# nikolovjovan/exblas

Measured on AMD Instinct MI355X. Metric: ExSUM fp64 Gelem/s at n=2^28 (bit-exact vs CPU superaccumulator/MPFR), higher is better.
Workload: dtype f64; 1 GPU; ExSUM n=2^28 fp64 ill_cond(c=1e+32), fpe=8 early_exit=True, 1xMI355X, inputs resident in HBM, steps rotate over 4 distinct vectors; n_total=268435456, fpe=8, early_exit=True, parallelism=single

## Files before the change

### exblas_amd/csrc/blas1.hip

```cpp
#include "superacc.hip.h"
#include "fpe.hip.h"
#include "exblas_internal.h"
#include <hip/hip_ext.h>

namespace exb {

constexpr int BLOCK = 256;
constexpr int WAVES = BLOCK / 64;

template <int N, bool EE, int COPIES, int CNT, int ZM = 0>
__device__ __forceinline__ void fpe_absorb(double (&a)[N > 0 ? N : 1], double (&x)[CNT], int from,
                                           long long *col, unsigned &flags)
{
    LdsSink<COPIES> sink{col, flags};
    fpe_absorb_sink<N, EE, CNT, LdsSink<COPIES>, ZM>(a, x, from, sink);
}

template <int N, int COPIES>
__device__ __forceinline__ void fpe_flush(double (&a)[N > 0 ? N : 1], long long *col, unsigned &flags)
{
    LdsSink<COPIES> sink{col, flags};
    fpe_flush_sink<N>(a, sink);
}

template <int COPIES>
__device__ __forceinline__ void block_epilogue(long long *s_acc, unsigned flags, long long *gacc,
                                               unsigned *gflags, int ngroups)
{
    __shared__ unsigned s_flags;
    if (threadIdx.x == 0) s_flags = 0;
    __syncthreads();
    if (flags) atomicOr(&s_flags, flags);
    long long *g = gacc + (size_t)(blockIdx.x % ngroups) * NL;
    for (int l = threadIdx.x; l < NL; l += BLOCK) {
        long long sum = 0;
#pragma unroll
        for (int w = 0; w < WAVES; ++w)
#pragma unroll
            for (int c = 0; c < COPIES; ++c) sum += s_acc[(w * NL + l) * COPIES + c];
        if (sum != 0) atomicAdd((unsigned long long *)&g[l], (unsigned long long)sum);
    }
    __syncthreads();
    if (threadIdx.x == 0 && s_flags) atomicOr(gflags, s_flags);
}

template <int N, bool EE, int COPIES, int U, bool NT, bool PF, int ZM = 0>
__global__ void __launch_bounds__(BLOCK) k_exsum(const double *__restrict__ a, long long n,
                                                 long long *__restrict__ gacc,
                                                 unsigned *__restrict__ gflags, int ngroups, int chunked)
{
    __shared__ long long s_acc[WAVES * NL * COPIES];
    auto zero_lds = [&]() {
        for (int i = threadIdx.x; i < WAVES * NL * COPIES; i += BLOCK) s_acc[i] = 0;
        __syncthreads();
    };
    const int wave = threadIdx.x >> 6, lane = threadIdx.x & 63;
    long long *col = s_acc + wave * NL * COPIES + (lane & (COPIES - 1));
    unsigned flags = 0;
    double fpe[N > 0 ? N : 1];
#pragma unroll
    for (int i = 0; i < (N > 0 ? N : 1); ++i) fpe[i] = 0.0;

    const long long head = (((uintptr_t)a & 8u) && n > 0) ? 1 : 0;
    const d2_t *v = (const d2_t *)(a + head);
    const long long nv = (n - head) >> 1;
    constexpr long long TILE = (long long)BLOCK * U;
    const long long ntiles = nv / TILE;
    LdsSink<COPIES> sinkm{col, flags};
    Bypass bypass;

    if constexpr (!PF) {
        zero_lds();
        for (long long t = blockIdx.x; t < ntiles; t += gridDim.x) {
            const d2_t *p = v + t * TILE + threadIdx.x;
            d2_t r[U];
#pragma unroll
            for (int u = 0; u < U; ++u) r[u] = ld2<NT>(p + u * BLOCK);
            double x[2 * U];
#pragma unroll
            for (int u = 0; u < U; ++u) {
                x[2 * u] = r[u].x;
                x[2 * u + 1] = r[u].y;
            }
            fpe_absorb_adaptive<N, EE, 2 * U, LdsSink<COPIES>, ZM>(fpe, x, sinkm, bypass);
        }
    } else {
        long long t = blockIdx.x, tstride = gridDim.x, tend = ntiles;
        if (chunked) {
            const long long per = (ntiles + gridDim.x - 1) / gridDim.x;
            t = blockIdx.x * per;
            tstride = 1;
            tend = min(ntiles, t + per);
        }
        if (t < tend) {
            d2_t r0[U], r1[U];
            auto fill = [&](long long tile, d2_t (&r)[U]) {
                const d2_t *p = v + (tile < tend ? tile : tend - 1) * TILE + threadIdx.x;
#pragma unroll
                for (int u = 0; u < U; ++u) r[u] = ld2<NT>(p + u * BLOCK);
            };
            auto absorb = [&](d2_t (&r)[U]) {
                double x[2 * U];
#pragma unroll
                for (int u = 0; u < U; ++u) {
                    x[2 * u] = r[u].x;
                    x[2 * u + 1] = r[u].y;
                }
                fpe_absorb_adaptive<N, EE, 2 * U, LdsSink<COPIES>, ZM>(fpe, x, sinkm, bypass);
            };
            fill(t, r0);
            zero_lds();
            for (;;) {
                fill(t + tstride, r1);
                absorb(r0);
                t += tstride;
                if (t >= tend) break;
                fill(t + tstride, r0);
                absorb(r1);
                t += tstride;
                if (t >= tend) break;
            }
        } else {
            zero_lds();
        }
    }
    for (long long i = ntiles * TILE + (long long)blockIdx.x * BLOCK + threadIdx.x; i < nv;
         i += (long long)gridDim.x * BLOCK) {
        d2_t r = v[i];
        double x[2] = {r.x, r.y};
        fpe_absorb<N, false, COPIES, 2>(fpe, x, 0, col, flags);
    }
    if (blockIdx.x == 0 && threadIdx.x == 0) {
        if (head) lds_add<COPIES>(col, a[0], flags);
        if ((n - head) & 1) lds_add<COPIES>(col, a[n - 1], flags);
    }
    fpe_flush<N, COPIES>(fpe, col, flags);
    block_epilogue<COPIES>(s_acc, flags, gacc, gflags, ngroups);
}

template <int N, bool EE, int COPIES>
__global__ void __launch_bounds__(BLOCK) k_exsum_strided(const double *__restrict__ a, long long n,
                                                         long long inca, long long *__restrict__ gacc,
                                                         unsigned *__restrict__ gflags, int ngroups)
{
    __shared__ long long s_acc[WAVES * NL * COPIES];
    for (int i = threadIdx.x; i < WAVES * NL * COPIES; i += BLOCK) s_acc[i] = 0;
    __syncthreads();
    const int wave = threadIdx.x >> 6, lane = threadIdx.x & 63;
    long long *col = s_acc + wave * NL * COPIES + (lane & (COPIES - 1));
    unsigned flags = 0;
    double fpe[N > 0 ? N : 1];
#pragma unroll
    for (int i = 0; i < (N > 0 ? N : 1); ++i) fpe[i] = 0.0;
    const long long T = (long long)gridDim.x * BLOCK;
    for (long long i = (long long)blockIdx.x * BLOCK + threadIdx.x; i < n; i += 4 * T) {
        double x[4];
#pragma unroll
        for (int u = 0; u < 4; ++u) x[u] = i + u * T < n ? a[(i + u * T) * inca] : 0.0;
        fpe_absorb<N, false, COPIES, 4>(fpe, x, 0, col, flags);
    }
    fpe_flush<N, COPIES>(fpe, col, flags);
    block_epilogue<COPIES>(s_acc, flags, gacc, gflags, ngroups);
}

template <int N, bool EE, int COPIES, int U, bool NT, bool PF, int WPS = 1, bool HALVES = false, int ZM = 0>
__global__ void __launch_bounds__(BLOCK, WPS) k_exdot(const double *__restrict__ a, const double *__restrict__ b,
                                                 long long n, long long *__restrict__ gacc,
                                                 unsigned *__restrict__ gflags, int ngroups)
{
    __shared__ long long s_acc[WAVES * NL * COPIES];
    auto zero_lds = [&]() {
        for (int i = threadIdx.x; i < WAVES * NL * COPIES; i += BLOCK) s_acc[i] = 0;
        __syncthreads();
    };
    const int wave = threadIdx.x >> 6, lane = threadIdx.x & 63;
    long long *col = s_acc + wave * NL * COPIES + (lane & (COPIES - 1));
    unsigned flags = 0;
    LdsSink<COPIES> sink{col, flags};
    long long *const lo_acc = low_acc_of(gflags), *const hi_acc = high_acc_of(gflags);
    double fpe[N > 0 ? N : 1];
#pragma unroll
    for (int i = 0; i < (N > 0 ? N : 1); ++i) fpe[i] = 0.0;

    const d2_t *va = (const d2_t *)a, *vb = (const d2_t *)b;
    const long long nv = n >> 1;
    Bypass bypass;
    constexpr long long TILE = (long long)BLOCK * U;
    const long long ntiles = nv / TILE;
    if constexpr (!PF) {
        zero_lds();
        for (long long t = blockIdx.x; t < ntiles; t += gridDim.x) {
            const long long base = t * TILE + threadIdx.x;
            d2_t ra[U], rb[U];
#pragma unroll
            for (int u = 0; u < U; ++u) {
                ra[u] = ld2<NT>(va + base + u * BLOCK);
                rb[u] = ld2<NT>(vb + base + u * BLOCK);
            }
            double x[2 * U], e[2 * U];
#pragma unroll
            for (int u = 0; u < U; ++u) {
                x[2 * u] = two_prod(ra[u].x, rb[u].x, e[2 * u]);
                x[2 * u + 1] = two_prod(ra[u].y, rb[u].y, e[2 * u + 1]);
            }
            if (!prod_range_divert<2 * U>(fpe[0], x, e, sink, lo_acc, hi_acc, [&](int j) { return j & 1 ? ra[j >> 1].y : ra[j >> 1].x; },
                                              [&](int j) { return j & 1 ? rb[j >> 1].y : rb[j >> 1].x; }))
                fpe_absorb_prod_adaptive<N, EE, 2 * U, LdsSink<COPIES>, 0, false>(fpe, x, e, sink, bypass);
        }
    } else {
        long long t = blockIdx.x;
        d2_t ra[U], rb[U];
        if (t < ntiles) {
            const long long base = t * TILE + threadIdx.x;
#pragma unroll
            for (int u = 0; u < U; ++u) {
                ra[u] = ld2<NT>(va + base + u * BLOCK);
                rb[u] = ld2<NT>(vb + base + u * BLOCK);
            }
        }
        zero_lds();
        if constexpr (HALVES) {
            while (t < ntiles) {
                const long long tn = t + gridDim.x;
                constexpr int H = U / 2;
#pragma unroll
                for (int h = 0; h < 2; ++h) {
                    double x[2 * H], e[2 * H];
#pragma unroll
                    for (int u = 0; u < H; ++u) {
                        x[2 * u] = two_prod(ra[h * H + u].x, rb[h * H + u].x, e[2 * u]);
                        x[2 * u + 1] = two_prod(ra[h * H + u].y, rb[h * H + u].y, e[2 * u + 1]);
                    }
                    const bool diverted = prod_range_divert<2 * H>(fpe[0], x, e, sink, lo_acc, hi_acc, [&](int j) { return j & 1 ? ra[h * H + (j >> 1)].y : ra[h * H + (j >> 1)].x; },
                        [&](int j) { return j & 1 ? rb[h * H + (j >> 1)].y : rb[h * H + (j >> 1)].x; });
                    if (tn < ntiles) {
                        const long long base = tn * TILE + threadIdx.x;
#pragma unroll
                        for (int u = 0; u < H; ++u) {
                            ra[h * H + u] = ld2<NT>(va + base + (h * H + u) * BLOCK);
                            rb[h * H + u] = ld2<NT>(vb + base + (h * H + u) * BLOCK);
                        }
                    }
                    if (!diverted) fpe_absorb_prod_adaptive<N, EE, 2 * H, LdsSink<COPIES>, 0, false>(fpe, x, e, sink, bypass);
                }
                t = tn;
            }
        } else if (t < ntiles) {
            d2_t rc[U], rd[U];
            auto fill = [&](long long tile, d2_t (&pa)[U], d2_t (&pb)[U]) {
                const long long base = (tile < ntiles ? tile : ntiles - 1) * TILE + threadIdx.x;
#pragma unroll
                for (int u = 0; u < U; ++u) {
                    pa[u] = ld2<NT>(va + base + u * BLOCK);
                    pb[u] = ld2<NT>(vb + base + u * BLOCK);
                }
            };
            auto absorb = [&](d2_t (&pa)[U], d2_t (&pb)[U]) {
                double x[2 * U], e[2 * U];
#pragma unroll
                for (int u = 0; u < U; ++u) {
                    x[2 * u] = two_prod(pa[u].x, pb[u].x, e[2 * u]);
                    x[2 * u + 1] = two_prod(pa[u].y, pb[u].y, e[2 * u + 1]);
                }
                if (!prod_range_divert<2 * U>(fpe[0], x, e, sink, lo_acc, hi_acc, [&](int j) { return j & 1 ? pa[j >> 1].y : pa[j >> 1].x; },
                                                  [&](int j) { return j & 1 ? pb[j >> 1].y : pb[j >> 1].x; }))
                    fpe_absorb_prod_adaptive<N, EE, 2 * U, LdsSink<COPIES>, ZM, false>(fpe, x, e, sink, bypass);
            };
            for (;;) {
                fill(t + gridDim.x, rc, rd);
                absorb(ra, rb);
                t += gridDim.x;
                if (t >= ntiles) break;
                fill(t + gridDim.x, ra, rb);
                absorb(rc, rd);
                t += gridDim.x;
                if (t >= ntiles) break;
            }
        }
    }
    for (long long i = ntiles * TILE + (long long)blockIdx.x * BLOCK + threadIdx.x; i < nv;
         i += (long long)gridDim.x * BLOCK) {
        d2_t ra = va[i], rb = vb[i];
        double x[2], e[2];
        x[0] = two_prod(ra.x, rb.x, e[0]);
        x[1] = two_prod(ra.y, rb.y, e[1]);
        if (!prod_range_divert<2>(fpe[0], x, e, sink, lo_acc, hi_acc, [&](int j) { return j ? ra.y : ra.x; }, [&](int j) { return j ? rb.y : rb.x; }))
            fpe_absorb_prod<N, false, 2, LdsSink<COPIES>, 0, false>(fpe, x, e, sink);
    }
    if (blockIdx.x == 0 && threadIdx.x == 0 && (n & 1)) {
        double x1[1], e1[1];
        x1[0] = two_prod(a[n - 1], b[n - 1], e1[0]);
        if (!prod_range_divert<1>(fpe[0], x1, e1, sink, lo_acc, hi_acc, [&](int) { return a[n - 1]; }, [&](int) { return b[n - 1]; }))
            sink_product(sink, x1[0], e1[0]);
    }
    fpe_flush<N, COPIES>(fpe, col, flags);
    block_epilogue<COPIES>(s_acc, flags, gacc, gflags, ngroups);
}

template <int N, bool EE, int COPIES>
__global__ void __launch_bounds__(BLOCK) k_exdot_strided(const double *__restrict__ a, long long inca,
                                                         const double *__restrict__ b, long long incb,
                                                         long long n, long long *__restrict__ gacc,
                                                         unsigned *__restrict__ gflags, int ngroups)
{
    __shared__ long long s_acc[WAVES * NL * COPIES];
    for (int i = threadIdx.x; i < WAVES * NL * COPIES; i += BLOCK) s_acc[i] = 0;
    __syncthreads();
    const int wave = threadIdx.x >> 6, lane = threadIdx.x & 63;
    long long *col = s_acc + wave * NL * COPIES + (lane & (COPIES - 1));
    unsigned flags = 0;
    LdsSink<COPIES> sink{col, flags};
    long long *const lo_acc = low_acc_of(gflags), *const hi_acc = high_acc_of(gflags);
    double fpe[N > 0 ? N : 1];
#pragma unroll
    for (int i = 0; i < (N > 0 ? N : 1); ++i) fpe[i] = 0.0;
    const long long T = (long long)gridDim.x * BLOCK;
    for (long long i = (long long)blockIdx.x * BLOCK + threadIdx.x; i < n; i += 4 * T) {
        double va[4], vb[4], x[4], e[4];
#pragma unroll
        for (int u = 0; u < 4; ++u) {
            const bool in = i + u * T < n;
            va[u] = in ? a[(i + u * T) * inca] : 0.0;
            vb[u] = in ? b[(i + u * T) * incb] : 0.0;
        }
#pragma unroll
        for (int u = 0; u < 4; ++u) x[u] = two_prod(va[u], vb[u], e[u]);
        if (!prod_range_divert<4>(fpe[0], x, e, sink, lo_acc, hi_acc, [&](int j) { return va[j]; }, [&](int j) { return vb[j]; }))
            fpe_absorb_prod<N, false, 4, LdsSink<COPIES>, 0, false>(fpe, x, e, sink);
    }
    fpe_flush<N, COPIES>(fpe, col, flags);
    block_epilogue<COPIES>(s_acc, flags, gacc, gflags, ngroups);
}

__global__ void __launch_bounds__(64) k_finalize(long long *sets, int nsets, int set_stride, unsigned *gflags,
                                                 unsigned flags_or, int zero_sets, long long *out,
                                                 const long long *ext_in, long long *ext_out)
{
    const int lane = threadIdx.x;
    unsigned flags = flags_or;
    if (gflags) flags |= *gflags;
    if (set_stride >= SET_WORDS) {
        for (int g = 0; g < nsets; ++g)
        {
            for (int k = 0; k < 3; ++k)
                if (sets[(size_t)g * set_stride + NL + k] != 0) flags |= (1u << k);
            const long long pw = sets[(size_t)g * set_stride + NL + 3];
            if (pw & 0xffff) flags |= FLAG_PUNDER;
            if (pw >> 16) flags |= FLAG_POVER;
        }
    }
    long long lo0 = 0, hi0 = 0, lo1 = 0, hi1 = 0;
    for (int g0 = 0; g0 < nsets; g0 += 16) {
        long long t0[16], t1[16];
#pragma unroll
        for (int k = 0; k < 16; ++k) {
            const bool ok = g0 + k < nsets;
            const long long *p = sets + (size_t)(ok ? g0 + k : 0) * set_stride;
            t0[k] = ok ? __builtin_nontemporal_load(p + lane) : 0;
            t1[k] = (ok && lane < NL - 64) ? __builtin_nontemporal_load(p + 64 + lane) : 0;
        }
#pragma unroll
        for (int k = 0; k < 16; ++k) {
            lo0 += t0[k] & 0xffffffffll;
            hi0 += t0[k] >> 32;
            if (lane == NL - 65) {
                lo1 += t1[k];
            } else {
                lo1 += t1[k] & 0xffffffffll;
                hi1 += t1[k] >> 32;
            }
        }
    }
    long long in0 = __shfl_up(hi0, 1), in1 = __shfl_up(hi1, 1);
    const long long h63 = __shfl(hi0, 63);
    if (lane == 0) { in0 = 0; in1 = h63; }
    long long v0 = lo0 + in0, v1 = (lane < NL - 64) ? lo1 + in1 : 0;
    if (zero_sets) {
        for (int i = lane; i < nsets * set_stride; i += 64) sets[i] = 0;
        if (lane == 0 && gflags) *gflags = 0;
    }
    __shared__ long long s_v[NL], s_lo[NL], s_hi[NL], s_c[NL + EXT_SHIFT_DIGITS];
    __shared__ unsigned long long s_ex;
    __shared__ int s_over;
    bool low_folded = false;
    const bool have_low = (flags & FLAG_PUNDER) && (ext_in || gflags);
    const bool have_high = (flags & FLAG_POVER) && (ext_in || gflags);
    if (ext_out) {
        if (!have_low) {
            ext_out[lane] = 0;
            if (lane < SET_WORDS - 64) ext_out[64 + lane] = 0;
        }
        if (!have_high) {
            ext_out[SET_WORDS + lane] = 0;
            if (lane < SET_WORDS - 64) ext_out[SET_WORDS + 64 + lane] = 0;
        }
    }
    if (have_low || have_high) {
        const long long *lsrc = ext_in ? ext_in : low_acc_of(gflags);
        const long long *hsrc = ext_in ? ext_in + SET_WORDS : high_acc_of(gflags);
        s_lo[lane] = have_low ? lsrc[lane] : 0;
        s_hi[lane] = have_high ? hsrc[lane] : 0;
        s_v[lane] = v0;
        if (lane < NL - 64) {
            s_lo[64 + lane] = have_low ? lsrc[64 + lane] : 0;
            s_hi[64 + lane] = have_high ? hsrc[64 + lane] : 0;
            s_v[64 + lane] = v1;
        }
        if (!ext_in && zero_sets) {
            long long *lo = low_acc_of(gflags), *hi = high_acc_of(gflags);
            if (have_low) {
                lo[lane] = 0;
                if (lane < NL - 64) lo[64 + lane] = 0;
            }
            if (have_high) {
                hi[lane] = 0;
                if (lane < NL - 64) hi[64 + lane] = 0;
            }
        }
        __syncthreads();
        if (lane == 0) {
            s_over = 0;
            if (have_low) normalize_digits(s_lo);
            if (have_high) normalize_digits(s_hi);
            if (!ext_out) {
                if (have_high) s_over = fold_high_digits(s_v, s_hi, s_c);
                if (have_low && !s_over) {
                    for (int j = LOW_SHIFT_DIGITS; j < NL; ++j) s_v[j - LOW_SHIFT_DIGITS] += s_lo[j];
                    normalize_digits(s_v);
                    const bool half = (s_lo[LOW_SHIFT_DIGITS - 1] >> 31) & 1ll;
                    bool sticky = (s_lo[LOW_SHIFT_DIGITS - 1] & 0x7fffffffll) != 0;
                    for (int j = 0; j < LOW_SHIFT_DIGITS - 1; ++j) sticky = sticky || s_lo[j] != 0;
                    s_ex = round_exact_bits_frac(s_v, half, sticky);
                }
            }
        }
        __syncthreads();
        if (ext_out) {
            if (have_low) {
                ext_out[lane] = s_lo[lane];
                if (lane < SET_WORDS - 64) ext_out[64 + lane] = lane < NL - 64 ? s_lo[64 + lane] : 0;
            }
            if (have_high) {
                ext_out[SET_WORDS + lane] = s_hi[lane];
                if (lane < SET_WORDS - 64) ext_out[SET_WORDS + 64 + lane] = lane < NL - 64 ? s_hi[64 + lane] : 0;
            }
        } else {
            const int over = s_over;
            if (over) {
                flags |= over > 0 ? FLAG_PINF : FLAG_NINF;
            } else {
                v0 = s_v[lane];
                v1 = lane < NL - 64 ? s_v[64 + lane] : 0;
                low_folded = have_low;
            }
            if (have_low) flags |= FLAG_PLOW_EXACT;
            if (have_high) flags |= FLAG_PHIGH_EXACT;
        }
    }
    WaveFinish r = finish_wave(v0, v1, flags);
    if (low_folded && !(flags & FLAG_NONFINITE)) r.ex = s_ex;
    write_record_wave(r, flags, out);
}

template <int N, bool EE>
__global__ void __launch_bounds__(BLOCK) k_exsum_segmented(const double *__restrict__ values,
                                                           const long long *__restrict__ offsets, long long nseg,
                                                           int round_mode, double *__restrict__ out)
{
    __shared__ long long acc[WAVES][NL];
    __shared__ unsigned fl[WAVES];
    const int lane = threadIdx.x & 63, w = threadIdx.x >> 6;
    const long long seg = (long long)blockIdx.x * WAVES + w;
    const bool valid = seg < nseg;
    for (int t = lane; t < NL; t += 64) acc[w][t] = 0;
    if (lane == 0) fl[w] = 0;
    __syncthreads();
    if (valid) {
        unsigned flags = 0;
        LdsSink<1> sink{acc[w], flags};
        double fpe[N > 0 ? N : 1];
#pragma unroll
        for (int i = 0; i < (N > 0 ? N : 1); ++i) fpe[i] = 0.0;
        const long long b = offsets[seg], e = offsets[seg + 1];
        for (long long i0 = b; i0 < e; i0 += 64) {
            const long long i = i0 + lane;
            double x[1] = {i < e ? values[i] : 0.0};
            fpe_absorb_sink<N, EE, 1>(fpe, x, 0, sink);
        }
        fpe_flush_sink<N>(fpe, sink);
        if (flags) atomicOr(&fl[w], flags);
    }
    __syncthreads();
    const WaveFinish r = finish_wave(acc[w][lane], lane < NL - 64 ? acc[w][64 + lane] : 0, fl[w]);
    if (valid && lane == 0) out[seg] = round_mode ? r.rf : __longlong_as_double((long long)r.ex);
}


#define EXB_LAUNCH_STREAMING(c, kernel, grid, st, ...)                                                                \
    do {                                                                                                               \
        if ((c).launch_stop_event || (c).launch_start_event) {                                                         \
            hipEvent_t ev0_ = (c).launch_start_event, ev1_ = (c).launch_stop_event;                                    \
            (c).launch_start_event = (c).launch_stop_event = nullptr;                                                  \
            hipExtLaunchKernelGGL(kernel, dim3(grid), dim3(BLOCK), 0, st, ev0_, ev1_, 0, __VA_ARGS__);                 \
        } else {                                                                                                       \
            hipLaunchKernelGGL(kernel, dim3(grid), dim3(BLOCK), 0, st, __VA_ARGS__);                                   \
        }                                                                                                              \
    } while (0)

static inline int grid_for(const Ctx &c, long long work_items, long long per_block, int blocks_per_cu)
{
    long long want = (work_items + per_block - 1) / per_block;
    long long cap = (long long)c.num_cu * blocks_per_cu;
    if (want < 1) want = 1;
    if (want >= cap) return (int)max(1ll, cap + c.grid_adj);
    return (int)want;
}

template <int N, bool EE, int COPIES, int U, bool NT, bool PF, int ZM = 0>
static void run_exsum(Ctx &c, const double *a, long long n, hipStream_t st)
{
    const int bpc = N == 0 ? c.bpc_sa : ((!SKIP_ZERO_LEVELS<EE> && N >= 5) ? c.bpc_heavy : c.bpc_sum);
    int grid = grid_for(c, n, (long long)BLOCK * 2 * U, bpc);
    if (grid == c.num_cu * bpc && grid > 1 && !(grid & 1)) grid -= 1;
    EXB_LAUNCH_STREAMING(c, (k_exsum<N, EE, COPIES, U, NT, PF, ZM>), grid, st, a, n, c.gacc, c.gflags, c.ngroups,
                         c.variant == 9 ? 1 : 0);
}

#ifndef EXBLAS_SUM_COPIES
#define EXBLAS_SUM_COPIES 8
#endif
#ifndef EXBLAS_DOT_COPIES
#define EXBLAS_DOT_COPIES 8
#endif
template <int N, bool EE>
static hipError_t launch_exsum(Ctx &c, const double *a, long long n, long long inca, hipStream_t st)
{
    constexpr int COPIES = (N == 0) ? 16 : EXBLAS_SUM_COPIES;
    if (inca == 1) {
        if constexpr (N == 8 && EE) {
            switch (c.variant) {
            case 1: run_exsum<N, EE, COPIES, 4, true, false>(c, a, n, st); break;
            case 2: run_exsum<N, EE, COPIES, 8, true, false>(c, a, n, st); break;
            case 3: run_exsum<N, EE, COPIES, 2, true, true>(c, a, n, st); break;
            case 4: run_exsum<N, EE, COPIES, 4, false, true>(c, a, n, st); break;
            case 5: run_exsum<N, EE, COPIES, 2, true, false>(c, a, n, st); break;
            case 6: run_exsum<N, EE, COPIES, 8, true, true>(c, a, n, st); break;
            case 7: run_exsum<N, EE, COPIES, 6, true, true>(c, a, n, st); break;
            case 8: run_exsum<N, EE, COPIES, 4, true, true, 1>(c, a, n, st); break;
            default: run_exsum<N, EE, COPIES, 4, true, true>(c, a, n, st); break;
            }
        } else {
            run_exsum<N, EE, COPIES, 4, true, true>(c, a, n, st);
        }
    } else {
        int grid = grid_for(c, n, BLOCK, c.blocks_per_cu);
        EXB_LAUNCH_STREAMING(c, (k_exsum_strided<N, EE, COPIES>), grid, st, a, n, inca, c.gacc, c.gflags, c.ngroups);
    }
    return hipGetLastError();
}

template <int N, bool EE, int COPIES, int U, bool NT, bool PF, int WPS = 1, bool HALVES = false, int ZM = 0>
static void run_exdot(Ctx &c, const double *a, const double *b, long long n, hipStream_t st)
{
    const long long tiles = n / ((long long)BLOCK * 2 * U);
    const int bpc = (int)min((long long)c.bpc_dot, max(4ll, tiles / (5ll * c.num_cu)));
    int grid = grid_for(c, n, (long long)BLOCK * 2 * U, bpc);
    if (grid > c.num_cu && !(grid & 1)) grid += 1;
    EXB_LAUNCH_STREAMING(c, (k_exdot<N, EE, COPIES, U, NT, PF, WPS, HALVES, ZM>), grid, st, a, b, n, c.gacc, c.gflags,
                         c.ngroups);
}

template <int N, bool EE>
static hipError_t launch_exdot(Ctx &c, const double *a, long long inca, const double *b, long long incb,
                               long long n, hipStream_t st)
{
    constexpr int COPIES = (N == 0) ? 16 : EXBLAS_DOT_COPIES;
    const bool vec = inca == 1 && incb == 1 && (((uintptr_t)a | (uintptr_t)b) & 15u) == 0;
    if (vec) {
        if constexpr (N == 8 && EE) {
            switch (c.variant) {
            case 1: run_exdot<N, EE, COPIES, 2, true, false>(c, a, b, n, st); break;
            case 2: run_exdot<N, EE, COPIES, 4, true, false>(c, a, b, n, st); break;
            case 3: run_exdot<N, EE, COPIES, 1, true, true>(c, a, b, n, st); break;
            case 4: run_exdot<N, EE, COPIES, 2, false, true>(c, a, b, n, st); break;
            case 5: run_exdot<N, EE, COPIES, 1, true, false>(c, a, b, n, st); break;
            case 6: run_exdot<N, EE, COPIES, 2, true, true>(c, a, b, n, st); break;
            case 7: run_exdot<N, EE, COPIES, 3, true, true>(c, a, b, n, st); break;
            case 8: run_exdot<N, EE, COPIES, 4, true, true, 1, true>(c, a, b, n, st); break;
            case 9: run_exdot<N, EE, COPIES, 8, true, true, 1, true>(c, a, b, n, st); break;
            case 10: run_exdot<N, EE, COPIES, 4, true, true>(c, a, b, n, st); break;
            default: run_exdot<N, EE, COPIES, 4, true, true, 1, false, 1>(c, a, b, n, st); break;
            }
        } else {
            run_exdot<N, EE, COPIES, 4, true, true, 1, false, SKIP_ZERO_LEVELS<EE> ? 1 : 0>(c, a, b, n, st);
        }
    } else {
        int grid = grid_for(c, n, BLOCK, c.blocks_per_cu);
        EXB_LAUNCH_STREAMING(c, (k_exdot_strided<N, EE, COPIES>), grid, st, a, inca, b, incb, n, c.gacc, c.gflags,
                             c.ngroups);
    }
    return hipGetLastError();
}

hipError_t finalize_groups(Ctx &c, hipStream_t st, long long *d_out, long long *d_ext_out)
{
    hipLaunchKernelGGL(k_finalize, dim3(1), dim3(64), 0, st, c.gacc, c.ngroups, NL, c.gflags, 0u, 1, d_out,
                       (const long long *)nullptr, d_ext_out);
    return hipGetLastError();
}

hipError_t finalize_sets(const long long *d_sets, int nsets, unsigned flags_or, hipStream_t st, long long *d_out,
                         const long long *d_ext_sets)
{
    hipLaunchKernelGGL(k_finalize, dim3(1), dim3(64), 0, st, const_cast<long long *>(d_sets), nsets, SET_WORDS,
                       (unsigned *)nullptr, flags_or, 0, d_out, d_ext_sets, (long long *)nullptr);
    return hipGetLastError();
}

hipError_t exsum_dispatch(Ctx &c, const double *a, long long n, long long inca, int fpe, int early_exit,
                          hipStream_t st, bool *supported)
{
    *supported = true;
    if (fpe < 2) return launch_exsum<0, false>(c, a, n, inca, st);
    if (early_exit) {
        if (fpe <= 4) return launch_exsum<4, true>(c, a, n, inca, st);
        if (fpe <= 6) return launch_exsum<6, true>(c, a, n, inca, st);
        if (fpe <= 8) return launch_exsum<8, true>(c, a, n, inca, st);
    } else {
        switch (fpe) {
        case 2: return launch_exsum<2, false>(c, a, n, inca, st);
        case 3: return launch_exsum<3, false>(c, a, n, inca, st);
        case 4: return launch_exsum<4, false>(c, a, n, inca, st);
        case 5: return launch_exsum<5, false>(c, a, n, inca, st);
        case 6: return launch_exsum<6, false>(c, a, n, inca, st);
        case 7: return launch_exsum<7, false>(c, a, n, inca, st);
        default: return launch_exsum<8, false>(c, a, n, inca, st);
        }
    }
    *supported = false;
    return hipSuccess;
}

hipError_t exsum_segmented_dispatch(const double *values, const long long *offsets, long long nseg, int fpe,
                                    int early_exit, int round_mode, hipStream_t st, double *out)
{
    if (nseg <= 0) return hipSuccess;
    const dim3 grid((unsigned)((nseg + WAVES - 1) / WAVES)), block(BLOCK);
#define SEG_GO(N, EE) \
    hipLaunchKernelGGL((k_exsum_segmented<N, EE>), grid, block, 0, st, values, offsets, nseg, round_mode, out)
    if (fpe < 2) SEG_GO(0, false);
    else if (early_exit) {
        if (fpe <= 4) SEG_GO(4, true);
        else if (fpe <= 6) SEG_GO(6, true);
        else if (fpe <= 8) SEG_GO(8, true);
        else return hipMemsetAsync(out, 0, sizeof(double) * nseg, st);
    } else {
        switch (fpe) {
        case 2: SEG_GO(2, false); break;
        case 3: SEG_GO(3, false); break;
        case 4: SEG_GO(4, false); break;
        case 5: SEG_GO(5, false); break;
        case 6: SEG_GO(6, false); break;
        case 7: SEG_GO(7, false); break;
        default: SEG_GO(8, false); break;
        }
    }
#undef SEG_GO
    return hipGetLastError();
}

hipError_t exdot_dispatch(Ctx &c, const double *a, long long inca, const double *b, long long incb, long long n,
                          int fpe, int early_exit, hipStream_t st, bool *supported)
{
    *supported = true;
    if (fpe < 3) return launch_exdot<0, false>(c, a, inca, b, incb, n, st);
    if (early_exit) {
        if (fpe <= 4) return launch_exdot<4, true>(c, a, inca, b, incb, n, st);
        if (fpe <= 6) return launch_exdot<6, true>(c, a, inca, b, incb, n, st);
        if (fpe <= 8) return launch_exdot<8, true>(c, a, inca, b, incb, n, st);
    } else {
        switch (fpe) {
        case 3: return launch_exdot<3, false>(c, a, inca, b, incb, n, st);
        case 4: return launch_exdot<4, false>(c, a, inca, b, incb, n, st);
        case 5: return launch_exdot<5, false>(c, a, inca, b, incb, n, st);
        case 6: return launch_exdot<6, false>(c, a, inca, b, incb, n, st);
        case 7: return launch_exdot<7, false>(c, a, inca, b, incb, n, st);
        default: return launch_exdot<8, false>(c, a, inca, b, incb, n, st);
        }
    }
    *supported = false;
    return hipSuccess;
}

}
```

Before: 865.0 Gelem/s.

## Parallelize finalize across four waves and speed up block epilogue merge

The single-wave finalize kernel now runs four waves. Each wave sums a strided subset of the group accumulators in batches of 32, gathers the per-set flag words with lane-parallel loads instead of a serial scalar loop, and zeroes the sets with 128-bit stores; the partial sums are then combined through LDS. The block epilogue reduces flags with wave shuffles and direct global atomicOr instead of an LDS atomic, and splits each limb's copy reduction across four lanes combined by shuffles. This targets the serial tail cost of the finalize launch and the epilogue, at the price of extra LDS, barriers and more complex wave-0-only control flow.

Result: no change. 867.9 Gelem/s, median of 6 (+0.3%).

```diff
diff --git a/exblas_amd/csrc/blas1.hip b/exblas_amd/csrc/blas1.hip
--- a/exblas_amd/csrc/blas1.hip
+++ b/exblas_amd/csrc/blas1.hip
@@ -27,21 +27,36 @@
 __device__ __forceinline__ void block_epilogue(long long *s_acc, unsigned flags, long long *gacc,
                                                unsigned *gflags, int ngroups)
 {
-    __shared__ unsigned s_flags;
-    if (threadIdx.x == 0) s_flags = 0;
+    static_assert(BLOCK == 4 * 64, "four lanes per limb");
+    if (__any(flags != 0)) {
+        for (int o = 1; o < 64; o <<= 1) flags |= __shfl_xor(flags, o);
+        if ((threadIdx.x & 63) == 0) atomicOr(gflags, flags);
+    }
     __syncthreads();
-    if (flags) atomicOr(&s_flags, flags);
+    constexpr int PART = COPIES >= 4 ? COPIES / 4 : 1;
+    const int j = threadIdx.x & 3;
+    auto merge = [&](int l) {
+        long long sum = 0;
+#pragma unroll
+        for (int w = 0; w < WAVES; ++w)
+#pragma unroll
+            for (int c = 0; c < PART; ++c)
+                if (COPIES >= 4 || j * PART + c < COPIES) sum += s_acc[(w * NL + l) * COPIES + j * PART + c];
+        sum += __shfl_xor(sum, 1);
+        sum += __shfl_xor(sum, 2);
+        return sum;
+    };
     long long *g = gacc + (size_t)(blockIdx.x % ngroups) * NL;
-    for (int l = threadIdx.x; l < NL; l += BLOCK) {
-        long long sum = 0;
-#pragma unroll
-        for (int w = 0; w < WAVES; ++w)
-#pragma unroll
-            for (int c = 0; c < COPIES; ++c) sum += s_acc[(w * NL + l) * COPIES + c];
-        if (sum != 0) atomicAdd((unsigned long long *)&g[l], (unsigned long long)sum);
-    }
-    __syncthreads();
-    if (threadIdx.x == 0 && s_flags) atomicOr(gflags, s_flags);
+    {
+        const int l = threadIdx.x >> 2;
+        const long long sum = merge(l);
+        if (j == 0 && sum != 0) atomicAdd((unsigned long long *)&g[l], (unsigned long long)sum);
+    }
+    if (threadIdx.x < 4 * (NL - 64)) {
+        const int l = 64 + (threadIdx.x >> 2);
+        const long long sum = merge(l);
+        if (j == 0 && sum != 0) atomicAdd((unsigned long long *)&g[l], (unsigned long long)sum);
+    }
 }
 
 template <int N, bool EE, int COPIES, int U, bool NT, bool PF, int ZM = 0>
@@ -332,52 +347,89 @@
     block_epilogue<COPIES>(s_acc, flags, gacc, gflags, ngroups);
 }
 
-__global__ void __launch_bounds__(64) k_finalize(long long *sets, int nsets, int set_stride, unsigned *gflags,
-                                                 unsigned flags_or, int zero_sets, long long *out,
-                                                 const long long *ext_in, long long *ext_out)
-{
-    const int lane = threadIdx.x;
+constexpr int FIN_WAVES = 4;
+constexpr int FIN_BATCH = 32;
+__global__ void __launch_bounds__(64 * FIN_WAVES) k_finalize(long long *sets, int nsets, int set_stride, unsigned *gflags,
+                                                             unsigned flags_or, int zero_sets, long long *out,
+                                                             const long long *ext_in, long long *ext_out)
+{
+    const int lane = threadIdx.x & 63, wave = __builtin_amdgcn_readfirstlane(threadIdx.x >> 6);
+    const bool record_sets = set_stride >= SET_WORDS;
+    const int words1 = record_sets ? SET_WORDS - 64 : NL - 64;
+    const unsigned *const gfp = (gflags ? gflags : (const unsigned *)out) + (lane & 15);
+    unsigned gfl = 0;
+    long long lo0 = 0, hi0 = 0, lo1 = 0, hi1 = 0;
+    unsigned fl = 0;
+    auto batch = [&](int g0, bool first) {
+        const int cnt = (nsets - g0 + FIN_WAVES - 1) / FIN_WAVES;
+        long long t0[FIN_BATCH], t1[FIN_BATCH];
+#pragma unroll
+        for (int k = 0; k < FIN_BATCH; ++k) {
+            t0[k] = t1[k] = 0;
+            if (k < cnt) {
+                const long long *p = sets + (size_t)(g0 + k * FIN_WAVES) * set_stride;
+                t0[k] = __builtin_nontemporal_load(p + lane);
+                if (lane < words1) t1[k] = __builtin_nontemporal_load(p + 64 + lane);
+            }
+        }
+        const unsigned gw = first ? __builtin_nontemporal_load(gfp) : 0u;
+#pragma unroll
+        for (int k = 0; k < FIN_BATCH; ++k) {
+            if (k < cnt) {
+                lo0 += t0[k] & 0xffffffffll;
+                hi0 += t0[k] >> 32;
+                if (lane == NL - 65) {
+                    lo1 += t1[k];
+                } else if (lane < NL - 64) {
+                    lo1 += t1[k] & 0xffffffffll;
+                    hi1 += t1[k] >> 32;
+                } else if (lane < NL - 61) {
+                    if (t1[k] != 0) fl |= 1u << (lane - (NL - 64));
+                } else if (lane == NL - 61) {
+                    if (t1[k] & 0xffff) fl |= FLAG_PUNDER;
+                    if (t1[k] >> 16) fl |= FLAG_POVER;
+                }
+            }
+        }
+        gfl |= gw;
+    };
+    if (wave < nsets) batch(wave, true);
+    for (int g0 = wave + FIN_WAVES * FIN_BATCH; g0 < nsets; g0 += FIN_WAVES * FIN_BATCH) batch(g0, false);
+    __shared__ long long s_part[FIN_WAVES][4][64];
+    __shared__ unsigned s_fl[FIN_WAVES];
+    fl |= __shfl_xor(fl, 1);
+    fl |= __shfl_xor(fl, 2);
+    fl |= __shfl_xor(fl, 4);
+    s_part[wave][0][lane] = lo0;
+    s_part[wave][1][lane] = hi0;
+    s_part[wave][2][lane] = lo1;
+    s_part[wave][3][lane] = hi1;
+    if (lane == 0) s_fl[wave] = fl | (gflags ? gfl : 0u);
+    if (zero_sets) {
+        const int words = nsets * set_stride;
+        for (int i = threadIdx.x; i < words / 2; i += 64 * FIN_WAVES)
+            reinterpret_cast<longlong2 *>(sets)[i] = make_longlong2(0, 0);
+        if (gflags && threadIdx.x == 0) *gflags = 0;
+    }
+    __syncthreads();
     unsigned flags = flags_or;
-    if (gflags) flags |= *gflags;
-    if (set_stride >= SET_WORDS) {
-        for (int g = 0; g < nsets; ++g)
-        {
-            for (int k = 0; k < 3; ++k)
-                if (sets[(size_t)g * set_stride + NL + k] != 0) flags |= (1u << k);
-            const long long pw = sets[(size_t)g * set_stride + NL + 3];
-            if (pw & 0xffff) flags |= FLAG_PUNDER;
-            if (pw >> 16) flags |= FLAG_POVER;
-        }
-    }
-    long long lo0 = 0, hi0 = 0, lo1 = 0, hi1 = 0;
-    for (int g0 = 0; g0 < nsets; g0 += 16) {
-        long long t0[16], t1[16];
-#pragma unroll
-        for (int k = 0; k < 16; ++k) {
-            const bool ok = g0 + k < nsets;
-            const long long *p = sets + (size_t)(ok ? g0 + k : 0) * set_stride;
-            t0[k] = ok ? __builtin_nontemporal_load(p + lane) : 0;
-            t1[k] = (ok && lane < NL - 64) ? __builtin_nontemporal_load(p + 64 + lane) : 0;
-        }
-#pragma unroll
-        for (int k = 0; k < 16; ++k) {
-            lo0 += t0[k] & 0xffffffffll;
-            hi0 += t0[k] >> 32;
-            if (lane == NL - 65) {
-                lo1 += t1[k];
-            } else {
-                lo1 += t1[k] & 0xffffffffll;
-                hi1 += t1[k] >> 32;
-            }
-        }
-    }
-    long long in0 = __shfl_up(hi0, 1), in1 = __shfl_up(hi1, 1);
-    const long long h63 = __shfl(hi0, 63);
-    if (lane == 0) { in0 = 0; in1 = h63; }
-    long long v0 = lo0 + in0, v1 = (lane < NL - 64) ? lo1 + in1 : 0;
-    if (zero_sets) {
-        for (int i = lane; i < nsets * set_stride; i += 64) sets[i] = 0;
-        if (lane == 0 && gflags) *gflags = 0;
+#pragma unroll
+    for (int w = 0; w < FIN_WAVES; ++w) flags |= s_fl[w];
+    long long v0 = 0, v1 = 0;
+    if (wave == 0) {
+        lo0 = hi0 = lo1 = hi1 = 0;
+#pragma unroll
+        for (int w = 0; w < FIN_WAVES; ++w) {
+            lo0 += s_part[w][0][lane];
+            hi0 += s_part[w][1][lane];
+            lo1 += s_part[w][2][lane];
+            hi1 += s_part[w][3][lane];
+        }
+        long long in0 = __shfl_up(hi0, 1), in1 = __shfl_up(hi1, 1);
+        const long long h63 = __shfl(hi0, 63);
+        if (lane == 0) { in0 = 0; in1 = h63; }
+        v0 = lo0 + in0;
+        v1 = (lane < NL - 64) ? lo1 + in1 : 0;
     }
     __shared__ long long s_v[NL], s_lo[NL], s_hi[NL], s_c[NL + EXT_SHIFT_DIGITS];
     __shared__ unsigned long long s_ex;
@@ -385,7 +437,7 @@
     bool low_folded = false;
     const bool have_low = (flags & FLAG_PUNDER) && (ext_in || gflags);
     const bool have_high = (flags & FLAG_POVER) && (ext_in || gflags);
-    if (ext_out) {
+    if (ext_out && wave == 0) {
         if (!have_low) {
             ext_out[lane] = 0;
             if (lane < SET_WORDS - 64) ext_out[64 + lane] = 0;
@@ -398,27 +450,29 @@
     if (have_low || have_high) {
         const long long *lsrc = ext_in ? ext_in : low_acc_of(gflags);
         const long long *hsrc = ext_in ? ext_in + SET_WORDS : high_acc_of(gflags);
-        s_lo[lane] = have_low ? lsrc[lane] : 0;
-        s_hi[lane] = have_high ? hsrc[lane] : 0;
-        s_v[lane] = v0;
-        if (lane < NL - 64) {
-            s_lo[64 + lane] = have_low ? lsrc[64 + lane] : 0;
-            s_hi[64 + lane] = have_high ? hsrc[64 + lane] : 0;
-            s_v[64 + lane] = v1;
-        }
-        if (!ext_in && zero_sets) {
-            long long *lo = low_acc_of(gflags), *hi = high_acc_of(gflags);
-            if (have_low) {
-                lo[lane] = 0;
-                if (lane < NL - 64) lo[64 + lane] = 0;
-            }
-            if (have_high) {
-                hi[lane] = 0;
-                if (lane < NL - 64) hi[64 + lane] = 0;
+        if (wave == 0) {
+            s_lo[lane] = have_low ? lsrc[lane] : 0;
+            s_hi[lane] = have_high ? hsrc[lane] : 0;
+            s_v[lane] = v0;
+            if (lane < NL - 64) {
+                s_lo[64 + lane] = have_low ? lsrc[64 + lane] : 0;
+                s_hi[64 + lane] = have_high ? hsrc[64 + lane] : 0;
+                s_v[64 + lane] = v1;
+            }
+            if (!ext_in && zero_sets) {
+                long long *lo = low_acc_of(gflags), *hi = high_acc_of(gflags);
+                if (have_low) {
+                    lo[lane] = 0;
+                    if (lane < NL - 64) lo[64 + lane] = 0;
+                }
+                if (have_high) {
+                    hi[lane] = 0;
+                    if (lane < NL - 64) hi[64 + lane] = 0;
+                }
             }
         }
         __syncthreads();
-        if (lane == 0) {
+        if (threadIdx.x == 0) {
             s_over = 0;
             if (have_low) normalize_digits(s_lo);
             if (have_high) normalize_digits(s_hi);
@@ -435,6 +489,7 @@
             }
         }
         __syncthreads();
+        if (wave != 0) return;
         if (ext_out) {
             if (have_low) {
                 ext_out[lane] = s_lo[lane];
@@ -457,6 +512,7 @@
             if (have_high) flags |= FLAG_PHIGH_EXACT;
         }
     }
+    if (wave != 0) return;
     WaveFinish r = finish_wave(v0, v1, flags);
     if (low_folded && !(flags & FLAG_NONFINITE)) r.ex = s_ex;
     write_record_wave(r, flags, out);
@@ -604,7 +660,7 @@
 
 hipError_t finalize_groups(Ctx &c, hipStream_t st, long long *d_out, long long *d_ext_out)
 {
-    hipLaunchKernelGGL(k_finalize, dim3(1), dim3(64), 0, st, c.gacc, c.ngroups, NL, c.gflags, 0u, 1, d_out,
+    hipLaunchKernelGGL(k_finalize, dim3(1), dim3(64 * FIN_WAVES), 0, st, c.gacc, c.ngroups, NL, c.gflags, 0u, 1, d_out,
                        (const long long *)nullptr, d_ext_out);
     return hipGetLastError();
 }
@@ -612,7 +668,7 @@
 hipError_t finalize_sets(const long long *d_sets, int nsets, unsigned flags_or, hipStream_t st, long long *d_out,
                          const long long *d_ext_sets)
 {
-    hipLaunchKernelGGL(k_finalize, dim3(1), dim3(64), 0, st, const_cast<long long *>(d_sets), nsets, SET_WORDS,
+    hipLaunchKernelGGL(k_finalize, dim3(1), dim3(64 * FIN_WAVES), 0, st, const_cast<long long *>(d_sets), nsets, SET_WORDS,
                        (unsigned *)nullptr, flags_or, 0, d_out, d_ext_sets, (long long *)nullptr);
     return hipGetLastError();
 }
```
